# hermda02/dang

Hardware: AMD Instinct MI355X
Metric: gibbs_iterations_per_sec (higher is better)
Workload: dtype f64

## Files before the change

dang_amd/csrc/dangx_core.hip:

```cpp
#include <dlfcn.h>

#include "dx_host.h"

DxRoctx::DxRoctx() {
    const char* e = getenv("DANGX_ROCTX");
    if (!(e && e[0] == '1')) return;
    for (const char* lib : {"librocprofiler-sdk-roctx.so", "libroctx64.so"}) {
        void* h = dlopen(lib, RTLD_NOW | RTLD_GLOBAL);
        if (!h) continue;
        push = reinterpret_cast<int (*)(const char*)>(dlsym(h, "roctxRangePushA"));
        pop = reinterpret_cast<int (*)()>(dlsym(h, "roctxRangePop"));
        if (push && pop) return;
        push = nullptr; pop = nullptr;
    }
}
const DxRoctx& dx_roctx() {
    static const DxRoctx r;
    return r;
}
const char* dx_kernel_family(int kid) {
    static const char* const names[DANGX_K_COUNT] = {"dangx:amplitude_solve", "dangx:index_sweep", "dangx:sky_chisq", "dangx:reduce",
                                                     "dangx:cg_Ax", "dangx:cg_vec", "dangx:solve+sweeps", "dangx:moments", "dangx:hist",
                                                     "dangx:signal", "dangx:chains", "dangx:batches"};
    return (kid >= 0 && kid < DANGX_K_COUNT) ? names[kid] : "dangx:?";
// ... 409 lines not shown
            for (size_t q = 0; q < nbp; ++q)
                if (ctx->bp_nu0[q] != 0.0) lnr[l * nbp + q] = std::log(ctx->bp_nu0[q] / ctx->desc[l].nu_ref);
        HIPCHK(ctx, hipMemcpy(ctx->d_bp_lnr, lnr.data(), nbytes * M.ncomp, hipMemcpyHostToDevice));
        ctx->bp_dirty = false;
    }
    M.bp_nu0 = ctx->d_bp_nu0; M.bp_tau0 = ctx->d_bp_tau0;
    for (int l = 0; l < M.ncomp; ++l) {
        Comp& c = M.comp[l];
        const dangx_comp_desc& d = ctx->desc[l];
        c.type = d.type; c.nind = d.nindices; c.group = d.cg_group; c.sample_amp = d.sample_amplitude;
        c.is_synch = d.is_synch; c.nu_ref = d.nu_ref;
        c.amp = ctx->amp[l]; c.idx = ctx->idx[l];
        c.tmpl = ctx->tmpl[l]; c.corr_mask = ctx->corr_mask[l]; c.nfit = ctx->nfit[l];
        c.bp_lnr = ctx->d_bp_lnr ? ctx->d_bp_lnr + (size_t)l * nbp : nullptr;
        for (int k = 0; k < 3; ++k)
            for (int j = 0; j < MAXB; ++j) c.tamp[k][j] = ctx->tamp[l][k][j];
        if (is_global_type(c.type) && !c.tmpl) return fail(ctx, "global-amplitude component without a template map (dangx_set_template)");
        for (int q = 0; q < MAXI; ++q) {
            c.lnl_type[q] = d.lnl_type[q]; c.prior_type[q] = d.prior_type[q];
            c.gauss[q][0] = d.gauss_prior[q][0]; c.gauss[q][1] = d.gauss_prior[q][1];
            c.uni[q][0] = d.uni_prior[q][0]; c.uni[q][1] = d.uni_prior[q][1];
            c.step[q] = d.step_size[q];
            c.lgden[q] = std::log(d.gauss_prior[q][1] * std::sqrt(2.0 * PI));
        }
        c.lnuref9 = std::log(1.0 * c.nu_ref / 1.0e9);
        for (int j = 0; j < M.nbands; ++j) {
            const double nu = M.band[j].nu_c;
            const double r = nu / c.nu_ref;
            c.lnr[j] = std::log(r);
            c.lnu9[j] = std::log(1.0 * nu / 1.0e9);
            c.cst[j] = 0.0;
            if (c.type == DANGX_CMB) c.cst[j] = 1.0 / host_a2t(ctx, j);
            else if (c.type == DANGX_FREEFREE) c.cst[j] = 1.0 / (r * r);
            else if (c.type == DANGX_LOGNORMAL) { const double q = c.nu_ref / nu; c.cst[j] = q * q; }
        }
        c.const_planes = 0;
        if (c.type >= DANGX_POWERLAW && c.type <= DANGX_CMB) {
            const unsigned cp = (c.nind == 0) ? 7u : ctx->idx_const[l];
            for (int k = 0; k < M.nmaps; ++k)
                if ((cp >> k) & 1) {
                    c.const_planes |= 1 << k;
                    const double t0 = ctx->idx_val[l][k][0], t1 = ctx->idx_val[l][k][1];
                    for (int j = 0; j < M.nbands; ++j) c.csed[k][j] = dx_host_band_sed(ctx, l, j, t0, t1);
                }
        }
    }
// ... 726 lines not shown
```

dang_amd/csrc/dangx_planeset.hip:

```cpp
#ifndef DX_NO_VCOEF
#define DX_VCOEF 1
#endif
#include "dx_host.h"
#include "dx_kern_planeset.h"

static int planeset_jeff(const SweepList& sl) {
    for (int q = 0; q < sl.n; ++q) if (sl.s[q].jeff) return 1;
    return 0;
}
static size_t planeset_lds(int ng, int nb, int nv, int lanes, int Sp, int jeff, int keep = 0) {
    const int rows = (nv > Sp + jeff ? nv : Sp + jeff) + (keep ? 1 : 0);
    return ((size_t)(TROWS * ng + 3) * nb + (size_t)rows * (nb / lanes) * BLOCK) * sizeof(double);
}

static int planeset_keep(const SweepList& sl, const FusedArgs& fa, int ng, int nb, int lanes, int Sp, int bp) {
#ifdef DX_BOUNDARY_REEVAL
    return 0;
#else
    if (lanes != 1 || bp || planeset_jeff(sl)) return 0;
    const int n = sl.n < 4 ? sl.n : 4;
    for (int q = 0; q < n; ++q) {
        if (sl.s[q].mode != CH_MBB_BETA) continue;
        const int v = fa.vslot[sl.s[q].gmember];
        if (v < 0 || planeset_lds(ng, nb, fa.nv, lanes, Sp, 0, 1) > 80u * 1024u) return 0;
        return (q > 0 && v >= Sp) ? 2 : 1;
    }
    return 0;
#endif
}

static void item_codes(const SweepList& sl, int code[4]) {
    for (int q = 0; q < 4; ++q) code[q] = (q < sl.n) ? sl.s[q].mode + 8 * sl.s[q].pair + 16 * (sl.s[q].jeff ? 1 : 0) : 0;
}
static std::string planeset_name(int Sp, int nb, int ng, int lanes, int solve, const SweepList& sl, int bp) {
    int c[4];
    item_codes(sl, c);
    std::string s = "dxk::k_plane_set<" + std::to_string(Sp) + ", " + std::to_string(nb) + ", " + std::to_string(ng) + ", " + std::to_string(lanes) +
                    ", " + std::to_string(solve);
    for (int q = 0; q < 4; ++q) s += ", " + std::to_string(c[q]);
    return s + ", " + std::to_string(bp) + ">";
}

static int planeset_bp(dangx_ctx* ctx) {
    for (int j = 0; j < ctx->hm.nbands; ++j)
        if (ctx->hm.band[j].n != 0) return 1;
    return 0;
}

static bool planeset_builtin(int nb, int ng, int lanes, int solve, const SweepList& sl) {
    if (const char* e = getenv("DANGX_PLANESET_RTC"); e && e[0] == '1' && dx_rtc_enabled()) return false;
    int c[4];
    item_codes(sl, c);
    if (solve == 2)
        return lanes == 1 && nb == 10 && ng == 4 && (sl.n == 0 || (c[0] == CH_POW && c[1] == CH_MBB_BETA + 8 && c[2] == 0 && c[3] == 0));
    if (nb == 20 && ng == 6 && lanes == 2) return solve && c[0] == CH_POW && c[1] == CH_MBB_BETA + 8 && c[2] == CH_LOGN_NUP && c[3] == 0;
    if (lanes == 1 && nb == 10 && ng == 4 && solve && sl.n == 0) return true;
// ... 59 lines not shown
    return true;
}

int dx_planeset_lanes(dangx_ctx* ctx, const GroupArgs& ga, const SweepList& sl, int solve_in) {
    const int solve = planeset_solve(ga, solve_in);
    static const bool enabled = [] { const char* e = getenv("DANGX_PLANESET"); return !(e && e[0] == '0'); }();
    static const bool small_too = [] { const char* e = getenv("DANGX_PLANESET"); return !(e && e[0] == 'p'); }();
    if (!enabled || sl.n < 0 || sl.n > 4 || (sl.n == 0 && !solve) || ga.ng < 1 || ga.ng > 6) return 0;
    static const int cap2 = [] { const char* e = getenv("DANGX_PS_CAP2"); return e ? atoi(e) : 13; }();
    const int nb = ctx->hm.nbands, Sp = sl.s2 - sl.s1 + 1, cap = (Sp == 2) ? cap2 : 16;
    for (int q = 0; q < sl.n; ++q) {
        const int m = sl.s[q].mode;
        if (m < CH_POW || m > CH_LOGN_W) return 0;
        if (sl.s[q].pair && !(m == CH_MBB_BETA || m == CH_LOGN_NUP)) return 0;
        if (sl.s[q].jeff && m != CH_POW) return 0;
    }
    FusedArgs fa;
    if (!planeset_args(ctx, ga, sl, fa)) return 0;
    if (solve && fa.cal && ga.nuc > 0) return 0;
    const int bp = planeset_bp(ctx), jf = planeset_jeff(sl);
    if (bp) {
        for (int q = 0; q < sl.n; ++q)
            if (sl.s[q].mode > CH_MBB_T || sl.s[q].jeff) return 0;
        if (!(small_too && nb <= cap && planeset_lds(ga.ng, nb, fa.nv, 1, Sp, 0) <= 80u * 1024u)) return 0;
        return dx_rtc_get(ctx, "dx_kern_planeset.h", planeset_name(Sp, nb, ga.ng, 1, solve, sl, 1)) ? 1 : 0;
    }
    int lanes = 0;
    if (small_too && nb <= cap && planeset_lds(ga.ng, nb, fa.nv, 1, Sp, jf) <= 80u * 1024u) lanes = 1;
    else if (nb > 12 && nb % 2 == 0 && nb / 2 <= cap && planeset_lds(ga.ng, nb, fa.nv, 2, Sp, jf) <= 80u * 1024u) lanes = 2;
    if (!lanes) return 0;
    if (planeset_builtin(nb, ga.ng, lanes, solve, sl)) return lanes;
    return dx_rtc_get(ctx, "dx_kern_planeset.h", planeset_name(Sp, nb, ga.ng, lanes, solve, sl, 0)) ? lanes : 0;
}

bool dx_launch_planeset(dangx_ctx* ctx, const GroupArgs& ga, const SweepList& sl_in, int lanes, int solve_in, unsigned nblk, unsigned long long* accp) {
    const int solve = planeset_solve(ga, solve_in);
    FusedArgs fa;
    if (lanes < 1 || lanes > 2 || !planeset_args(ctx, ga, sl_in, fa)) return false;
    SweepList sl = sl_in;
    const int nb = ctx->hm.nbands, ng = ga.ng, Sp = sl.s2 - sl.s1 + 1;
    const int bp = planeset_bp(ctx);
    sl.keep = planeset_keep(sl, fa, ng, nb, lanes, Sp, bp);
    const size_t ldsz = planeset_lds(ng, nb, fa.nv, lanes, Sp, planeset_jeff(sl), sl.keep);
    if (!bp && planeset_builtin(nb, ng, lanes, solve, sl)) {
        if (solve == 2) dx_launch_planeset_fluct(ctx, ga, fa, sl, Sp, nblk, ldsz, accp);
        else if (planeset_jeff(sl)) dx_launch_planeset_jeff(ctx, ga, fa, sl, Sp, solve, nblk, ldsz, accp);
        else if (nb == 20) launch_builtin<20, 6, 2, 1, CH_POW, CH_MBB_BETA + 8, CH_LOGN_NUP>(ctx, ga, fa, sl, Sp, nblk, ldsz, accp);
        else if (nb == 10 && sl.n == 0) launch_builtin<10, 4, 1, 1, 0, 0, 0>(ctx, ga, fa, sl, Sp, nblk, ldsz, accp);
        else if (nb == 10 && !solve) launch_builtin<10, 4, 1, 0, CH_POW, CH_MBB_BETA + 8, 0>(ctx, ga, fa, sl, Sp, nblk, ldsz, accp);
        else if (nb == 10) launch_builtin<10, 4, 1, 1, CH_POW, CH_MBB_BETA + 8, 0>(ctx, ga, fa, sl, Sp, nblk, ldsz, accp);
        else if (nb == 5) launch_builtin<5, 3, 1, 1, CH_POW, CH_MBB_BETA + 8, 0>(ctx, ga, fa, sl, Sp, nblk, ldsz, accp);
        else launch_builtin<3, 2, 1, 1, CH_POW, CH_MBB_BETA + 8, 0>(ctx, ga, fa, sl, Sp, nblk, ldsz, accp);
        return true;
    }
    hipFunction_t fn = dx_rtc_get(ctx, "dx_kern_planeset.h", planeset_name(Sp, nb, ng, lanes, solve, sl, bp));
    if (!fn) return false;
    const Model* dm = ctx->dm;
    GroupArgs gg = ga;
    SweepList ss = sl;
    unsigned long long* bad = ctx->counters;
    double* part = ctx->partial;
    void* args[] = {&dm, &gg, &fa, &ss, &bad, &accp, &part};
    return dx_rtc_launch(ctx, fn, nblk, ldsz, args) == 0;
}

#endif
// ... 9 lines not shown
```

dang_amd/csrc/dx_chain.h:

```cpp
#pragma once
#include "dx_args.h"


template <bool V> struct BoolTag { static constexpr bool value = V; };

#ifdef DX_CHAIN_LIBEXP
#define CEXP(x) exp(x)
#define CEXPS(x) exp(x)
#define CEXPA(x) exp(x)
#define CEXP1(x) exp(x)
#else
#define CEXP(x) exp_nr(x)
#define CEXPS(x) exp_sat(x)
#define CEXPA(x) exp_any(x)
#define CEXP1(x) exp_nr_v(x)
#endif
#ifdef DX_CHAIN_IEEEDIV
#define CDIV(a, b) ((a) / (b))
#define CDIVE(a, b) ((a) / (b))
#define CRCPE(b) (1.0 / (b))
#else
#define CDIV(a, b) ((a) * fast_rcp(b))
#define CDIVE(a, b) ((a) * fast_rcp_ends(b))
#define CRCPE(b) fast_rcp_ends(b)
// ... 64 lines not shown

#ifdef DX_LNL_DIAG
__device__ unsigned long long g_lnl_diag[2];
__device__ __forceinline__ void lnl_diag_count(int k) {
    if (__lane_id() == __builtin_ctzll(__builtin_amdgcn_ballot_w64(true))) atomicAdd(&g_lnl_diag[k], 1ull);
}
#endif

template <int LP>
struct BandPick {
    int half;
    __device__ __forceinline__ double operator()(const double* arr, int j, int nbh) const {
        if (LP == 1) return arr[j];
        const double a = arr[j], b = arr[nbh + j];
        return half ? b : a;
    }
    __device__ __forceinline__ double nu_c(const Model& M, int j, int nbh) const {
        if (LP == 1) return M.band[j].nu_c;
        const double a = M.band[j].nu_c, b = M.band[nbh + j].nu_c;
        return half ? b : a;
    }
};

template <int MODE, int SP, int NB, int LP, bool KT = false, bool BP = false, bool JF = false, bool KEPT = false>
struct RegChain {
    static constexpr bool kBP = BP;
    static constexpr bool kJF = JF;
    static constexpr bool kKept = KEPT;
    static_assert(!KEPT || (LP == 1 && !BP && !JF && (MODE == CH_MBB_BETA || MODE == CH_MBB_T)), "kept factors: one-lane delta-band mbb chains");
    static_assert(!JF || (MODE == CH_POW && !BP), "Jeffreys chains: power law, delta bands");
    double D[SP][NB], F[NB], ISr[SP][NB];
    double bpa, bpb;
    double K1[(LP > 1 && !KT) ? NB : 1], K2[(LP > 1 && !KT) ? NB : 1];
    const double *kt1, *kt2;
    double amp[SP];
    double W[(JF && !KT) ? NB : 1], jS;
    double* wcol;
    const double* fcol;

    __device__ __forceinline__ double w(int j) const { return KT ? wcol[j * BLOCK] : W[j]; }
    template <class ISF>
    __device__ __forceinline__ void form_w(const Model& M, const Comp& c, ISF is_of) {
        bool bad = false;
#pragma unroll
        for (int kk = 0; kk < SP; ++kk) bad = bad || !(fabs(amp[kk]) > 0.0 && fabs(amp[kk]) < INFINITY);
#pragma unroll
        for (int j = 0; j < NB; ++j) {
            const double t0 = is_of(0, j) * is_of(0, j);
            double q = t0 * t0;
            if (SP == 2) { const double t1 = is_of(SP - 1, j) * is_of(SP - 1, j); q = fma(t1, t1, q); }
            const double l = k1(M, c, j);
            const double wj = bad ? __longlong_as_double(0x7ff8000000000000ll) : (l * l) * q;
            if (KT) wcol[j * BLOCK] = wj; else W[j] = wj;
        }
    }
    __device__ __forceinline__ void jeff_eval(const Model& M, const Comp& c, double th) {
        double S = 0.0;
#pragma unroll
        for (int j = 0; j < NB; ++j) { const double e = CEXP(th * k1(M, c, j)); S = fma(e * e, w(j), S); }
        if (LP > 1) S += __shfl_xor(S, 1, 64);
        jS = S;
    }

    __device__ __forceinline__ double is(int kk, int j) const { return ISr[kk][j]; }
    __device__ __forceinline__ void set_is(int kk, int j, double v) { ISr[kk][j] = v; }
    __device__ __forceinline__ double k1(const Model& M, const Comp& c, int j) const {
        if (KT) return kt1[j];
        if (LP > 1) return K1[j];
        return (MODE == CH_MBB_T) ? M.band[j].nu_c : (MODE == CH_LOGN_NUP) ? c.lnu9[j] : c.lnr[j];
    }
    __device__ __forceinline__ double k2(const Comp& c, int j) const { return KT ? kt2[j] : (LP > 1) ? K2[j] : c.cst[j]; }
    __device__ __forceinline__ void set_kt(const double* tab, int nbands, int ng, int g, int jb) {
        kt1 = tab + ((MODE == CH_MBB_T) ? TROWS * ng : (MODE == CH_LOGN_NUP) ? TROWS * g + 2 : TROWS * g) * nbands + jb;
        kt2 = tab + (TROWS * g + 1) * nbands + jb;
    }
    __device__ __forceinline__ void set_k(const Model& M, const Comp& c, const BandPick<LP>& pick) {
        if (LP > 1 && !KT) {
#pragma unroll
            for (int j = 0; j < NB; ++j) {
                K1[j] = (MODE == CH_MBB_T) ? pick.nu_c(M, j, NB) : (MODE == CH_LOGN_NUP) ? pick(c.lnu9, j, NB) : pick(c.lnr, j, NB);
                K2[j] = (MODE == CH_LOGN_NUP || MODE == CH_LOGN_W) ? pick(c.cst, j, NB) : 0.0;
            }
        }
    }

    template <bool BATCH, int OP = 0, bool EOUT = false>
    __device__ __forceinline__ double lnl(const Model& M, const Comp& c, double th, double other, double& acc0, double& acc1,
                                          double* eout = nullptr) {
        static_assert(!EOUT || (MODE == CH_MBB_BETA && !BP), "the exported factor is the beta chain's");
        double s0 = 0.0, s1 = 0.0;
        if (MODE == CH_POW) s0 = th;
        else if (MODE == CH_MBB_BETA) s0 = th + 1.0;
        else if (MODE == CH_MBB_T) { s0 = mbb_z(th); s1 = CEXP(s0 * c.nu_ref) - 1.0; }
        else if (MODE == CH_LOGN_NUP) { s0 = log_pos(th); s1 = other; }
        else s1 = th;
        acc0 = 0.0; acc1 = 0.0;
        double S = 0.0;
#ifdef DX_CHAIN_IEEEDIV
// ... 135 lines not shown
        else if (MODE == CH_MBB_BETA) s0 = th + 1.0;
        else { s0 = mbb_z(th); s1 = CEXP(s0 * c.nu_ref) - 1.0; }
        const double s0l = s0 * 0x1.71547652b82fep+0;
        double acc0 = 0.0, acc1 = 0.0;
#pragma unroll
        for (int j = 0; j < NB; ++j) {
            const float e = __builtin_amdgcn_exp2f((float)(s0l * k1(M, c, j)));
            double s;
            if (MODE == CH_POW) s = (double)e;
            else if (MODE == CH_MBB_BETA) s = F[j] * (double)e;
            else s = (s1 * F[j]) * (double)__builtin_amdgcn_rcpf(e - 1.0f);
            const double r0 = fma(-is(0, j), s, D[0][j]);
            acc0 = fma(r0, r0, acc0);
            if (SP == 2) {
                const double r1 = fma(-is(SP - 1, j), s, D[SP - 1][j]);
                acc1 = fma(r1, r1, acc1);
            }
        }
        double a = acc0 + acc1;
        if (LP > 1) a += __shfl_xor(a, 1, 64);
        return a;
    }

    __device__ __forceinline__ bool cheap_bound(const Model& M, const Comp& c, double lo, double hi, double a_start,
                                                double& wA, double& wG) {
        double G = 0.0, emax = 0.0, kmax = 0.0;
        double smax, zmin = 0.0;
        if (MODE == CH_POW) smax = fmax(fabs(lo), fabs(hi));
        else if (MODE == CH_MBB_BETA) smax = fmax(fabs(lo + 1.0), fabs(hi + 1.0));
        else { smax = mbb_z(lo); zmin = mbb_z(hi); }
#pragma unroll
        for (int j = 0; j < NB; ++j) {
            const double k = fabs(k1(M, c, j));
            kmax = fmax(kmax, k);
            double e;
            if (MODE == CH_MBB_T) e = (1.0 + smax * k) * 0x1p-24 + (2.0 + (double)__builtin_amdgcn_rcpf((float)(zmin * k))) * 0x1p-22;
            else e = (smax * k) * 0x1p-24 + 0x1p-22;
            e = e * (1.0 + 0x1p-8) + 0x1p-46;
            emax = fmax(emax, e);
#pragma unroll
            for (int kk = 0; kk < SP; ++kk) { const double t = e * D[kk][j]; G = fma(t, t, G); }
        }
        if (LP > 1) { G += __shfl_xor(G, 1, 64); emax = fmax(emax, __shfl_xor(emax, 1, 64)); kmax = fmax(kmax, __shfl_xor(kmax, 1, 64)); }
        const double lam = fmax(sqrt(G * fast_rcp(fmax(a_start, 0x1p-900))), 0x1p-400);
        wA = 0.5 * ((2.0 * emax * (1.0 + emax) + lam) * (1.0 + 0x1p-40) + 0x1p-40);
        wG = 0.5 * ((G * fast_rcp(lam) + 2.0 * G) * (1.0 + 0x1p-40) + 0x1p-1000);
        const bool range = smax * kmax * 0x1.71547652b82fep+0 <= 125.0;
        return (MODE == CH_MBB_T) ? (range && lo > 0.0 && zmin > 0.0) : range;
    }
    __device__ __forceinline__ void scale() {
#ifdef DX_CHAIN_SCALED
#pragma unroll
        for (int kk = 0; kk < SP; ++kk)
#pragma unroll
            for (int j = 0; j < NB; ++j) { D[kk][j] *= ISr[kk][j]; ISr[kk][j] *= amp[kk]; }
#endif
    }
};

template <int NB, int LP>
__device__ __forceinline__ void subtract_other(const Model& M, const Comp& c2, int k, double amp2, double t0, double t1,
                                               double (&Dk)[NB], const BandPick<LP>& pick) {
    if ((c2.const_planes >> (k - 1)) & 1) {
#pragma unroll
        for (int j = 0; j < NB; ++j) Dk[j] -= amp2 * pick(c2.csed[k - 1], j, NB);
        return;
    }
    const Prep pr = sed_prep(c2, t0, t1);
    switch (c2.type) {
    case DANGX_POWERLAW:
#pragma unroll
// ... 85 lines not shown
    } else if (MODE == CH_MBB_T && RC::kKept) {
    } else if (MODE == CH_MBB_BETA) {
        const double z = mbb_z(sample1);
        const double A = CEXP(z * c.nu_ref) - 1.0;
#pragma unroll
        for (int j = 0; j < NB; ++j) R.F[j] = CDIVE(A, CEXP(z * pick.nu_c(M, j, NB)) - 1.0);
        if (RC::kBP) { R.bpa = z; R.bpb = A; }
    } else if (MODE == CH_MBB_T) {
#pragma unroll
        for (int j = 0; j < NB; ++j) R.F[j] = CEXP((sample0 + 1.0) * pick(c.lnr, j, NB));
        if (RC::kBP) R.bpa = sample0 + 1.0;
    } else if (MODE == CH_LOGN_W) {
        {
            const double lp = log_pos(sample0);
#pragma unroll
            for (int j = 0; j < NB; ++j) R.F[j] = pick(c.lnu9, j, NB) - lp;
        }
    }
    const double other = first ? sample1 : sample0;
    const unsigned long long gpix = (unsigned long long)(M.pix0 + i);
    const int q = a.nind;
    const bool gauss = c.prior_type[q] == DANGX_PRIOR_GAUSSIAN;
    const double pmean = c.gauss[q][0], pstd = c.gauss[q][1], lgden = c.lgden[q];
    const double inv2v = 1.0 / (2 * (pstd * pstd));
    auto prior = [&](double v) -> double {
        if (!gauss) return 0.0;
#ifdef DX_CHAIN_IEEEDIV
        const double arg = ((v - pmean) * (v - pmean)) / (2 * (pstd * pstd));
#else
        const double arg = ((v - pmean) * (v - pmean)) * inv2v;
#endif
        return (arg > 745.0) ? -INFINITY : -arg - lgden;
    };
    auto jprior = [&](double S) -> double {
        double p = log_pos(sqrt(S));
        if (!(S >= 0x1p-1022 && S < INFINITY)) p = log(sqrt(S));
        return p;
    };
    unsigned long long nacc = 0;
    double cur = first ? sample0 : sample1;
    double a0, a1, c0, c1;
    const double step = c.step[q], lo = c.uni[q][0], hi = c.uni[q][1];
    const bool ml_opt = (a.ml_mode == DANGX_ML_OPTIMIZE);
#if defined(DX_LNL_EXACT) || !defined(DX_CHAIN_SCALED)
    constexpr bool kCert = false;
#else
    constexpr bool kCert = !RC::kBP && !JEFF && (MODE == CH_POW || MODE == CH_MBB_BETA || MODE == CH_MBB_T);
#endif
    auto chain = [&](auto batch_tag) {
        constexpr bool B = decltype(batch_tag)::value;
        double lnl;
        if (acc_in) { a0 = acc_in[0]; a1 = acc_in[1]; lnl = a0 + a1; if (JEFF) R.jeff_eval(M, c, cur); }
        else if constexpr (ADD && RC::kKept) {
            if (scol) lnl = R.lnl_add_kept(scol, a0, a1);
            else lnl = R.template lnl<B, 1>(M, c, cur, other, a0, a1);
        }
        else lnl = R.template lnl<B, ADD ? 1 : 0>(M, c, cur, other, a0, a1);
        chi[0] = -2.0 * a0; chi[1] = -2.0 * a1;
        double lnl_old = lnl + (JEFF ? jprior(R.jS) : prior(cur));
        bool cert = false, old_exact = true, sums_exact = true;
        double wA = 0.0, wG = 0.0, wold = 0.0;
        if (kCert) {
            const bool ok = R.cheap_bound(M, c, lo, hi, -2.0 * lnl, wA, wG) && !ml_opt;
            cert = __builtin_amdgcn_ballot_w64(!ok) == 0ull;
        }
        auto mh_step = [&](double prop, uint32_t u3) {
            if (prop < lo || prop > hi) return;
            if constexpr (!kCert) {
                lnl = R.template lnl<B>(M, c, prop, other, c0, c1);
                const double lnl_new = lnl + (JEFF ? jprior(R.jS) : prior(prop));
                const double diff = lnl_new - lnl_old;
                const bool acc = ml_opt ? (diff > 0.0) : mh_accept(diff, u3);
                if (acc) { cur = prop; lnl_old = lnl_new; a0 = c0; a1 = c1; ++nacc; }
            } else {
                const double pp = prior(prop);
                bool acc = false, und = true;
                double lc = 0.0, wc = 0.0;
                if (cert) {
                    const double A = R.lnl_cheap(M, c, prop);
                    lc = -0.5 * A;
                    wc = fma(wA, A, wG);
                    const double dc = (lc + pp) - lnl_old;
                    const double W = (wc + wold) * (1.0 + 0x1p-40) + 0x1p-49 * ((fabs(lc) + fabs(pp)) + fabs(lnl_old));
                    und = !mh_certain(dc - W, dc + W, u3, acc);
#ifdef DX_LNL_DIAG
                    lnl_diag_count(0);
// ... 212 lines not shown
```

dang_amd/csrc/dx_kern_planeset.h:

```cpp
#pragma once
#include "dx_kern_fused.h"

#ifndef DX_PS_WAVES
#define DX_PS_WAVES(SP, NB, LP, SOLVE, C0) (((NB) / (LP) <= 5) ? 3 : 2)
#endif

namespace dxk {

template <int V> struct ItemCode { static constexpr int value = V; };
template <bool V> struct ItemFlag { static constexpr bool value = V; };

#ifdef DX_BOUNDARY_REEVAL
#define DX_PS_SHARE(MODE, LP, BP, JF) false
#else
#define DX_PS_SHARE(MODE, LP, BP, JF) ((MODE) == CH_MBB_BETA && (LP) == 1 && !(BP) && !(JF))
#endif
template <int MODE, int PAIR, int SP, int NBL, int LP, int NG, bool FIRST, bool LAST, bool BP, bool JF, typename RFirst>
__device__ __forceinline__ void ps_item(const Model& M, const SweepList& sl, const SweepItem& it, RFirst& R0, int i, int half,
                                        int jb, int NB, const double* __restrict__ tab, const double* __restrict__ col,
                                        double& sample0, double& sample1, double chi_first[4],
                                        double chi_last[4], unsigned int* __restrict__ accepted, int slot, const double* first_acc,
                                        double* wrow, const double* fkeep, const double* skeep) {
    const Comp& c = M.comp[it.comp];
    const BandPick<LP> pick = {half};
    const int npix = M.npix;
    IndexArgs a;
    a.comp = it.comp; a.nind = it.nind; a.s1 = sl.s1; a.s2 = sl.s2; a.nsample = sl.nsample; a.ml_mode = sl.ml_mode; a.mode = MODE;
    a.bp = 0; a.others = 0u; a.jeff = 0; a.seed = sl.seed; a.stream = it.stream;
    constexpr bool SHARE = DX_PS_SHARE(MODE, LP, BP, JF);
    RegChain<MODE, SP, NBL, LP, true, BP, JF, SHARE> R;
    R.set_kt(tab, NB, NG, it.gmember, jb);
    R.fcol = fkeep;
#pragma unroll
    for (int kk = 0; kk < SP; ++kk) {
        R.amp[kk] = c.amp[(long long)(sl.s1 + kk - 1) * npix + i];
#pragma unroll
        for (int j = 0; j < NBL; ++j) { R.D[kk][j] = R0.D[kk][j]; R.ISr[kk][j] = col[(kk * NBL + j) * BLOCK] * R.amp[kk]; }
    }
    if (JF) {
        R.wcol = wrow;
        R.form_w(M, c, [&](int kk, int j) { return col[(kk * NBL + j) * BLOCK]; });
    }
    double chia[4] = {0.0, 0.0, 0.0, 0.0}, va, acc[2];
    constexpr bool HAND = SHARE && PAIR != 0;
    double ej[HAND ? NBL : 1];
    unsigned long long na = chain_finish<MODE, SP, NBL, LP, false, !FIRST, (!PAIR && !LAST), HAND>(M, a, c, R, pick, sample0, sample1, i, half, chia, &va,
                                                                                                  FIRST ? first_acc : nullptr, acc, ej, skeep);
    if (it.nind == 0) sample0 = va; else sample1 = va;
    if (FIRST) { chi_first[0] = chia[0]; chi_first[1] = chia[1]; }
    chi_last[2] = chia[2]; chi_last[3] = chia[3];
    unsigned long long nb_ = 0ull;
    if (PAIR) {
        constexpr int MODEB = (MODE == CH_MBB_BETA || MODE == CH_LOGN_NUP) ? MODE + 1 : MODE;
        RegChain<MODEB, SP, NBL, LP, true, BP, false, HAND> RB;
        RB.set_kt(tab, NB, NG, it.gmember, jb);
        if (HAND) {
#pragma unroll
            for (int j = 0; j < NBL; ++j) RB.F[j] = ej[j];
        }
#pragma unroll
        for (int kk = 0; kk < SP; ++kk) {
            RB.amp[kk] = R.amp[kk];
#pragma unroll
            for (int j = 0; j < NBL; ++j) { RB.D[kk][j] = R.D[kk][j]; RB.ISr[kk][j] = R.ISr[kk][j]; }
        }
        IndexArgs b = a;
        b.nind = it.nind + 1; b.stream = it.stream2; b.mode = MODEB;
        double chib[4] = {0.0, 0.0, 0.0, 0.0}, vb;
        nb_ = chain_finish<MODEB, SP, NBL, LP, false, false, !LAST>(M, b, c, RB, pick, sample0, sample1, i, half, chib, &vb, acc);
        if (b.nind == 0) sample0 = vb; else sample1 = vb;
        chi_last[2] = chib[2]; chi_last[3] = chib[3];
        if (!LAST) {
#pragma unroll
            for (int kk = 0; kk < SP; ++kk)
#pragma unroll
                for (int j = 0; j < NBL; ++j) R0.D[kk][j] = RB.D[kk][j];
        }
    } else if (!LAST) {
#pragma unroll
        for (int kk = 0; kk < SP; ++kk)
#pragma unroll
            for (int j = 0; j < NBL; ++j) R0.D[kk][j] = R.D[kk][j];
    }
    if (accepted) {
        const int copy = threadIdx.x & 15;
        if (na) atomicAdd(accepted + (slot << 4) + copy, (unsigned int)na);
        if (nb_) atomicAdd(accepted + ((slot + 1) << 4) + copy, (unsigned int)nb_);
    }
}

template <int SP, int NB, int NG, int LP, int SOLVE, int C0, int C1, int C2, int C3, int BP = 0>
__global__ __launch_bounds__(BLOCK, DX_PS_WAVES(SP, NB, LP, SOLVE, C0)) void k_plane_set(const Model* __restrict__ Mp, GroupArgs ga, FusedArgs fa, SweepList sl,
                                                        unsigned long long* __restrict__ not_spd, unsigned long long* __restrict__ accepted,
                                                        double* __restrict__ chi_partial) {
    constexpr int NBL = NB / LP;
    extern __shared__ double lds[];
    const Model& M = *Mp;
    const int npix = M.npix, tid = threadIdx.x;
    double* tab = lds;
    double* col = lds + (TROWS * NG + 3) * NB + tid;
    const long long t0 = (long long)blockIdx.x * BLOCK + tid;
    const long long u = t0 / LP;
    const int half = (int)(t0 % LP), jb = half * NBL;
    const bool in_range = u < npix;
    const int i = in_range ? (int)u : 0;
    const double mk = M.mask[i];
    sed_table_build(M, tab, tid, BLOCK, ga.gc, NG);
    __shared__ unsigned int acc_blk[DX_MAX_IDXSUM * 16];
    if (tid < DX_MAX_IDXSUM * 16) acc_blk[tid] = 0u;
    __syncthreads();
    double chi[4] = {0.0, 0.0, 0.0, 0.0};
    constexpr int NS0 = C0 ? 1 + ((C0 >> 3) & 1) : 0, NS1 = C1 ? 1 + ((C1 >> 3) & 1) : 0, NS2 = C2 ? 1 + ((C2 >> 3) & 1) : 0, NS3 = C3 ? 1 + ((C3 >> 3) & 1) : 0;
    constexpr int NS = NS0 + NS1 + NS2 + NS3;
    const bool live = in_range && !is_masked(mk);
    if (in_range && !live && half == 0) {
        for (int q = 0; q < sl.n; ++q) {
            const Comp& c = M.comp[sl.s[q].comp];
            for (int e = 0; e <= sl.s[q].pair; ++e) {
                double* out = c.idx + ((long long)(sl.s[q].nind + e) * M.nmaps) * npix + i;
#pragma unroll
                for (int kk = 0; kk < SP; ++kk) out[(long long)(sl.s1 + kk - 1) * npix] = 0.0;
            }
        }
    }
    if (live) {
        const long long bstride = (long long)M.nmaps * npix;
        const unsigned long long gpix = (unsigned long long)(M.pix0 + i);
        const bool sample = (ga.ml_mode == DANGX_ML_SAMPLE);
        constexpr int KQ = ((C0 & 7) == CH_MBB_BETA) ? 0 : ((C1 & 7) == CH_MBB_BETA) ? 1 : ((C2 & 7) == CH_MBB_BETA) ? 2 : 3;
        constexpr bool KEEPC = DX_PS_SHARE(CH_MBB_BETA, LP, BP, false) &&
// ... 193 lines not shown
                const SweepItem it0 = sl.s[0];
                const double* m = col + (fa.vslot[it0.gmember] * NBL) * BLOCK;
#pragma unroll
                for (int kk = 0; kk < SP; ++kk) {
                    const double a0 = M.comp[it0.comp].amp[(long long)(sl.s1 + kk - 1) * npix + i];
                    double acc = 0.0;
#pragma unroll
                    for (int j = 0; j < NBL; ++j) {
                        const double r = R0.D[kk][j];
                        acc = fma(r, r, acc);
                        R0.D[kk][j] = fma(a0 * R0.ISr[kk][j], m[j * BLOCK], r);
                    }
                    if (LP > 1) acc += __shfl_xor(acc, 1, 64);
                    first_acc[kk] = -0.5 * acc;
                }
            }
#pragma unroll
            for (int kk = 0; kk < SP; ++kk)
#pragma unroll
                for (int j = 0; j < NBL; ++j) col[(kk * NBL + j) * BLOCK] = R0.ISr[kk][j];
            __builtin_amdgcn_sched_barrier(0);
        }
        int slot = 0;
        auto run = [&](auto code_tag, auto first_tag, auto last_tag, int q) {
            constexpr int CODE = decltype(code_tag)::value;
            constexpr bool FIRST = decltype(first_tag)::value;
            constexpr bool LAST = decltype(last_tag)::value;
            if constexpr (CODE != 0) {
                const SweepItem it = sl.s[q];
                const Comp& c = M.comp[it.comp];
                double sample0, sample1, unused[4];
                load_theta(M, c, i, sl.s1, sample0, sample1);
                ps_item<(CODE & 7), ((CODE >> 3) & 1), SP, NBL, LP, NG, FIRST, LAST, (BP != 0), ((CODE >> 4) != 0)>(M, sl, it, R0, i, half, jb, NB, tab, col, sample0, sample1,
                                                                              FIRST ? chi : unused, chi, accepted ? acc_blk : nullptr, slot, first_acc,
                                                                              col + (SP * NBL) * BLOCK, (KEEPC && q == KQ) ? fkeep : nullptr,
                                                                              (KEEPC && q == KQ) ? skeep : nullptr);
                slot += 1 + ((CODE >> 3) & 1);
            }
        };
        run(ItemCode<C0>{}, ItemFlag<true>{}, ItemFlag<C1 == 0>{}, 0);
        run(ItemCode<C1>{}, ItemFlag<false>{}, ItemFlag<C2 == 0>{}, 1);
        run(ItemCode<C2>{}, ItemFlag<false>{}, ItemFlag<C3 == 0>{}, 2);
        run(ItemCode<C3>{}, ItemFlag<false>{}, ItemFlag<true>{}, 3);
    }
    if (accepted && NS > 0) {
        __syncthreads();
        if (tid < NS) {
            unsigned int v = 0u;
            for (int q = 0; q < 16; ++q) v += acc_blk[(tid << 4) + q];
            if (v != 0u) atomicAdd(accepted + tid, (unsigned long long)v);
        }
    }
    if (chi_partial) {
        double isum[NS > 0 ? NS : 1];
#pragma unroll
        for (int q = 0; q < (NS > 0 ? NS : 1); ++q) isum[q] = 0.0;
        if (live && half == 0) {
            constexpr int code[4] = {C0, C1, C2, C3};
            constexpr int first[4] = {0, NS0, NS0 + NS1, NS0 + NS1 + NS2};
#pragma unroll
            for (int q = 0; q < 4; ++q)
                if (code[q] != 0) {
                    const double* at = M.comp[sl.s[q].comp].idx + ((long long)sl.s[q].nind * M.nmaps + (sl.s1 - 1)) * npix + i;
                    isum[first[q]] = at[0];
                    if (((code[q] >> 3) & 1) != 0) isum[first[q] + 1] = at[(long long)M.nmaps * npix];
                }
// ... 19 lines not shown
```

dang_amd/csrc/dx_model.h:

```cpp
#pragma once
#include "dx_rtc_compat.h"
#ifdef __HIPCC_RTC__
#include "dangx.h"
#else
#include "../../include/dangx.h"
#endif

namespace dx {

constexpr int MAXB = DANGX_MAX_BANDS;
constexpr int MAXC = DANGX_MAX_COMPS;
constexpr int MAXI = DANGX_MAX_IND;
constexpr int MAXG = DANGX_MAX_GROUP;
constexpr int MAXT = 4;

constexpr double PI = 3.141592653589793238462643383279502884197;
constexpr double K_B = 1.3806503e-23;
constexpr double C_LIGHT = 2.99792458e8;
constexpr double MISSVAL = -1.6375e30;
constexpr double H_PLANCK = 1.0545726691251021e-34 * 2.0 * PI;

__host__ __device__ inline double mbb_z(double T) {
    const double z = H_PLANCK / (K_B * T);
    return z > 1e-4 ? 1e-4 : (z < -1e-4 ? -1e-4 : z);
}

struct Band {
    double nu_c;
    int n;
    int off;
};

struct Comp {
    int type, nind, group, sample_amp, is_synch, pad;
    double nu_ref;
    double* amp;
    double* idx;
    int lnl_type[MAXI], prior_type[MAXI];
    double gauss[MAXI][2], uni[MAXI][2], step[MAXI];
    double lgden[MAXI];
    double lnr[MAXB];
    double cst[MAXB];
    double lnu9[MAXB];
    double lnuref9;
    int const_planes, pad1;
    double csed[3][MAXB];
    const double* tmpl;
    int corr_mask, nfit;
    double tamp[3][MAXB];
    const double* bp_lnr;
};

struct Model {
    int npix, nmaps, nbands, ncomp;
    int all_delta, pad0;
    long long pix0;
    const double* sig;
    const double* rms;
    const double* mask;
    const double* bp_nu0;
    const double* bp_tau0;
    double tcmb;
    double mbb_batch_z;
// ... 10 lines not shown
```

Measured before the change: 102.2.

## Precompute per-block certification error rows in LDS and host-side prior inverse variance

Builds a per-item certification row (per-band error bounds, max error and a range verdict) once per block in shared memory using one wavefront per row, instead of every lane recomputing the bounds from the component's prior range in each chain. The per-lane cheap bound then just reads these rows, and the held K1 coefficients are copied into registers. The Gaussian prior's inverse double variance is also precomputed on the host and stored in Comp rather than divided per call. This trades extra LDS footprint, which can push configurations over the lane or LDS thresholds, and more registers for less per-lane arithmetic.

```diff
diff --git a/dang_amd/csrc/dangx_core.hip b/dang_amd/csrc/dangx_core.hip
--- a/dang_amd/csrc/dangx_core.hip
+++ b/dang_amd/csrc/dangx_core.hip
@@ -455,6 +455,7 @@
             c.uni[q][0] = d.uni_prior[q][0]; c.uni[q][1] = d.uni_prior[q][1];
             c.step[q] = d.step_size[q];
             c.lgden[q] = std::log(d.gauss_prior[q][1] * std::sqrt(2.0 * PI));
+            c.inv2v[q] = prior_inv2v(d.gauss_prior[q][1]);
         }
         c.lnuref9 = std::log(1.0 * c.nu_ref / 1.0e9);
         for (int j = 0; j < M.nbands; ++j) {
diff --git a/dang_amd/csrc/dangx_planeset.hip b/dang_amd/csrc/dangx_planeset.hip
--- a/dang_amd/csrc/dangx_planeset.hip
+++ b/dang_amd/csrc/dangx_planeset.hip
@@ -8,9 +8,19 @@
     for (int q = 0; q < sl.n; ++q) if (sl.s[q].jeff) return 1;
     return 0;
 }
-static size_t planeset_lds(int ng, int nb, int nv, int lanes, int Sp, int jeff, int keep = 0) {
+static size_t planeset_lds(int ng, int nb, int nv, int lanes, int Sp, int jeff, int ncert, int keep = 0) {
     const int rows = (nv > Sp + jeff ? nv : Sp + jeff) + (keep ? 1 : 0);
-    return ((size_t)(TROWS * ng + 3) * nb + (size_t)rows * (nb / lanes) * BLOCK) * sizeof(double);
+    return ((size_t)(TROWS * ng + 3) * nb + (size_t)ncert * cert_row_size(nb) + (size_t)rows * (nb / lanes) * BLOCK) * sizeof(double);
+}
+
+static void item_codes(const SweepList& sl, int code[4]) {
+    for (int q = 0; q < 4; ++q) code[q] = (q < sl.n) ? sl.s[q].mode + 8 * sl.s[q].pair + 16 * (sl.s[q].jeff ? 1 : 0) : 0;
+}
+static int planeset_cert(const SweepList& sl, int bp) {
+    int c[4], n = 0;
+    item_codes(sl, c);
+    for (int q = 0; q < 4; ++q) n += dxk::ps_cert_rows(c[q], bp);
+    return n;
 }
 
 static int planeset_keep(const SweepList& sl, const FusedArgs& fa, int ng, int nb, int lanes, int Sp, int bp) {
@@ -22,16 +32,13 @@
     for (int q = 0; q < n; ++q) {
         if (sl.s[q].mode != CH_MBB_BETA) continue;
         const int v = fa.vslot[sl.s[q].gmember];
-        if (v < 0 || planeset_lds(ng, nb, fa.nv, lanes, Sp, 0, 1) > 80u * 1024u) return 0;
+        if (v < 0 || planeset_lds(ng, nb, fa.nv, lanes, Sp, 0, planeset_cert(sl, bp), 1) > 80u * 1024u) return 0;
         return (q > 0 && v >= Sp) ? 2 : 1;
     }
     return 0;
 #endif
 }
 
-static void item_codes(const SweepList& sl, int code[4]) {
-    for (int q = 0; q < 4; ++q) code[q] = (q < sl.n) ? sl.s[q].mode + 8 * sl.s[q].pair + 16 * (sl.s[q].jeff ? 1 : 0) : 0;
-}
 static std::string planeset_name(int Sp, int nb, int ng, int lanes, int solve, const SweepList& sl, int bp) {
     int c[4];
     item_codes(sl, c);
@@ -137,12 +144,13 @@
     if (bp) {
         for (int q = 0; q < sl.n; ++q)
             if (sl.s[q].mode > CH_MBB_T || sl.s[q].jeff) return 0;
-        if (!(small_too && nb <= cap && planeset_lds(ga.ng, nb, fa.nv, 1, Sp, 0) <= 80u * 1024u)) return 0;
+        if (!(small_too && nb <= cap && planeset_lds(ga.ng, nb, fa.nv, 1, Sp, 0, 0) <= 80u * 1024u)) return 0;
         return dx_rtc_get(ctx, "dx_kern_planeset.h", planeset_name(Sp, nb, ga.ng, 1, solve, sl, 1)) ? 1 : 0;
     }
+    const int nc = planeset_cert(sl, 0);
     int lanes = 0;
-    if (small_too && nb <= cap && planeset_lds(ga.ng, nb, fa.nv, 1, Sp, jf) <= 80u * 1024u) lanes = 1;
-    else if (nb > 12 && nb % 2 == 0 && nb / 2 <= cap && planeset_lds(ga.ng, nb, fa.nv, 2, Sp, jf) <= 80u * 1024u) lanes = 2;
+    if (small_too && nb <= cap && planeset_lds(ga.ng, nb, fa.nv, 1, Sp, jf, nc) <= 80u * 1024u) lanes = 1;
+    else if (nb > 12 && nb % 2 == 0 && nb / 2 <= cap && planeset_lds(ga.ng, nb, fa.nv, 2, Sp, jf, nc) <= 80u * 1024u) lanes = 2;
     if (!lanes) return 0;
     if (planeset_builtin(nb, ga.ng, lanes, solve, sl)) return lanes;
     return dx_rtc_get(ctx, "dx_kern_planeset.h", planeset_name(Sp, nb, ga.ng, lanes, solve, sl, 0)) ? lanes : 0;
@@ -156,7 +164,7 @@
     const int nb = ctx->hm.nbands, ng = ga.ng, Sp = sl.s2 - sl.s1 + 1;
     const int bp = planeset_bp(ctx);
     sl.keep = planeset_keep(sl, fa, ng, nb, lanes, Sp, bp);
-    const size_t ldsz = planeset_lds(ng, nb, fa.nv, lanes, Sp, planeset_jeff(sl), sl.keep);
+    const size_t ldsz = planeset_lds(ng, nb, fa.nv, lanes, Sp, planeset_jeff(sl), planeset_cert(sl, bp), sl.keep);
     if (!bp && planeset_builtin(nb, ng, lanes, solve, sl)) {
         if (solve == 2) dx_launch_planeset_fluct(ctx, ga, fa, sl, Sp, nblk, ldsz, accp);
         else if (planeset_jeff(sl)) dx_launch_planeset_jeff(ctx, ga, fa, sl, Sp, solve, nblk, ldsz, accp);
diff --git a/dang_amd/csrc/dx_chain.h b/dang_amd/csrc/dx_chain.h
--- a/dang_amd/csrc/dx_chain.h
+++ b/dang_amd/csrc/dx_chain.h
@@ -110,21 +110,70 @@
     }
 };
 
+template <int MODE>
+__device__ __forceinline__ void cert_range(double lo, double hi, double& smax, double& zmin) {
+    zmin = 0.0;
+    if (MODE == CH_POW) smax = fmax(fabs(lo), fabs(hi));
+    else if (MODE == CH_MBB_BETA) smax = fmax(fabs(lo + 1.0), fabs(hi + 1.0));
+    else { smax = mbb_z(lo); zmin = mbb_z(hi); }
+}
+template <int MODE>
+__device__ __forceinline__ double cert_band(double smax, double zmin, double k) {
+    double e;
+    if (MODE == CH_MBB_T) e = (1.0 + smax * k) * 0x1p-24 + (2.0 + (double)__builtin_amdgcn_rcpf((float)(zmin * k))) * 0x1p-22;
+    else e = (smax * k) * 0x1p-24 + 0x1p-22;
+    return e * (1.0 + 0x1p-8) + 0x1p-46;
+}
+template <int MODE>
+__device__ __forceinline__ bool cert_verdict(double lo, double smax, double zmin, double kmax) {
+    const bool range = smax * kmax * 0x1.71547652b82fep+0 <= 125.0;
+    return (MODE == CH_MBB_T) ? (range && lo > 0.0 && zmin > 0.0) : range;
+}
+constexpr int CERT_EMAX = 0, CERT_OK = 1, CERT_TAIL = 2;
+__host__ __device__ constexpr int cert_row_size(int nb) { return nb + CERT_TAIL; }
+template <int MODE>
+__device__ __forceinline__ void cert_row_build(const Model& M, const Comp& c, int q, int nb, double* row, int tid, int wave) {
+    if ((tid >> 6) != wave) return;
+    const int lane = tid & 63;
+    const double lo = c.uni[q][0], hi = c.uni[q][1];
+    double smax, zmin;
+    cert_range<MODE>(lo, hi, smax, zmin);
+    const int j = lane < nb ? lane : nb - 1;
+    const double k = fabs((MODE == CH_MBB_T) ? M.band[j].nu_c : c.lnr[j]);
+    const double e = cert_band<MODE>(smax, zmin, k);
+    if (lane < nb) row[lane] = e;
+    double emax = e, kmax = k;
+    for (int o = 32; o > 0; o >>= 1) { emax = fmax(emax, __shfl_xor(emax, o, 64)); kmax = fmax(kmax, __shfl_xor(kmax, o, 64)); }
+    emax = fmax(emax, 0.0); kmax = fmax(kmax, 0.0);
+    if (lane == 0) {
+        row[nb + CERT_EMAX] = emax;
+        row[nb + CERT_OK] = cert_verdict<MODE>(lo, smax, zmin, kmax) ? 1.0 : 0.0;
+    }
+}
+
 template <int MODE, int SP, int NB, int LP, bool KT = false, bool BP = false, bool JF = false, bool KEPT = false>
 struct RegChain {
     static constexpr bool kBP = BP;
     static constexpr bool kJF = JF;
     static constexpr bool kKept = KEPT;
+#ifdef DX_CERT_PER_LANE
+    static constexpr bool kCertRow = false;
+#else
+    static constexpr bool kCertRow = KT;
+#endif
+    static constexpr bool kCertified = !BP && !JF && (MODE == CH_POW || MODE == CH_MBB_BETA || MODE == CH_MBB_T);
+    static constexpr bool kHeld = kCertRow && kCertified;
     static_assert(!KEPT || (LP == 1 && !BP && !JF && (MODE == CH_MBB_BETA || MODE == CH_MBB_T)), "kept factors: one-lane delta-band mbb chains");
     static_assert(!JF || (MODE == CH_POW && !BP), "Jeffreys chains: power law, delta bands");
     double D[SP][NB], F[NB], ISr[SP][NB];
     double bpa, bpb;
-    double K1[(LP > 1 && !KT) ? NB : 1], K2[(LP > 1 && !KT) ? NB : 1];
+    double K1[((LP > 1 && !KT) || kHeld) ? NB : 1], K2[(LP > 1 && !KT) ? NB : 1];
     const double *kt1, *kt2;
     double amp[SP];
     double W[(JF && !KT) ? NB : 1], jS;
     double* wcol;
     const double* fcol;
+    const double *cej, *ctail;
 
     __device__ __forceinline__ double w(int j) const { return KT ? wcol[j * BLOCK] : W[j]; }
     template <class ISF>
@@ -153,6 +202,7 @@
     __device__ __forceinline__ double is(int kk, int j) const { return ISr[kk][j]; }
     __device__ __forceinline__ void set_is(int kk, int j, double v) { ISr[kk][j] = v; }
     __device__ __forceinline__ double k1(const Model& M, const Comp& c, int j) const {
+        if (kHeld) return K1[j];
         if (KT) return kt1[j];
         if (LP > 1) return K1[j];
         return (MODE == CH_MBB_T) ? M.band[j].nu_c : (MODE == CH_LOGN_NUP) ? c.lnu9[j] : c.lnr[j];
@@ -161,7 +211,12 @@
     __device__ __forceinline__ void set_kt(const double* tab, int nbands, int ng, int g, int jb) {
         kt1 = tab + ((MODE == CH_MBB_T) ? TROWS * ng : (MODE == CH_LOGN_NUP) ? TROWS * g + 2 : TROWS * g) * nbands + jb;
         kt2 = tab + (TROWS * g + 1) * nbands + jb;
-    }
+        if (kHeld) {
+#pragma unroll
+            for (int j = 0; j < NB; ++j) K1[j] = kt1[j];
+        }
+    }
+    __device__ __forceinline__ void set_cert(const double* row, int nbands, int jb) { cej = row + jb; ctail = row + nbands; }
     __device__ __forceinline__ void set_k(const Model& M, const Comp& c, const BandPick<LP>& pick) {
         if (LP > 1 && !KT) {
 #pragma unroll
@@ -343,31 +398,40 @@
         return a;
     }
 
+    __device__ __forceinline__ void cheap_widths(double G, double emax, double a_start, double& wA, double& wG) const {
+        const double lam = fmax(sqrt(G * fast_rcp(fmax(a_start, 0x1p-900))), 0x1p-400);
+        wA = 0.5 * ((2.0 * emax * (1.0 + emax) + lam) * (1.0 + 0x1p-40) + 0x1p-40);
+        wG = 0.5 * ((G * fast_rcp(lam) + 2.0 * G) * (1.0 + 0x1p-40) + 0x1p-1000);
+    }
     __device__ __forceinline__ bool cheap_bound(const Model& M, const Comp& c, double lo, double hi, double a_start,
                                                 double& wA, double& wG) {
         double G = 0.0, emax = 0.0, kmax = 0.0;
-        double smax, zmin = 0.0;
-        if (MODE == CH_POW) smax = fmax(fabs(lo), fabs(hi));
-        else if (MODE == CH_MBB_BETA) smax = fmax(fabs(lo + 1.0), fabs(hi + 1.0));
-        else { smax = mbb_z(lo); zmin = mbb_z(hi); }
+        double smax, zmin;
+        cert_range<MODE>(lo, hi, smax, zmin);
 #pragma unroll
         for (int j = 0; j < NB; ++j) {
             const double k = fabs(k1(M, c, j));
             kmax = fmax(kmax, k);
-            double e;
-            if (MODE == CH_MBB_T) e = (1.0 + smax * k) * 0x1p-24 + (2.0 + (double)__builtin_amdgcn_rcpf((float)(zmin * k))) * 0x1p-22;
-            else e = (smax * k) * 0x1p-24 + 0x1p-22;
-            e = e * (1.0 + 0x1p-8) + 0x1p-46;
+            const double e = cert_band<MODE>(smax, zmin, k);
             emax = fmax(emax, e);
 #pragma unroll
             for (int kk = 0; kk < SP; ++kk) { const double t = e * D[kk][j]; G = fma(t, t, G); }
         }
         if (LP > 1) { G += __shfl_xor(G, 1, 64); emax = fmax(emax, __shfl_xor(emax, 1, 64)); kmax = fmax(kmax, __shfl_xor(kmax, 1, 64)); }
-        const double lam = fmax(sqrt(G * fast_rcp(fmax(a_start, 0x1p-900))), 0x1p-400);
-        wA = 0.5 * ((2.0 * emax * (1.0 + emax) + lam) * (1.0 + 0x1p-40) + 0x1p-40);
-        wG = 0.5 * ((G * fast_rcp(lam) + 2.0 * G) * (1.0 + 0x1p-40) + 0x1p-1000);
-        const bool range = smax * kmax * 0x1.71547652b82fep+0 <= 125.0;
-        return (MODE == CH_MBB_T) ? (range && lo > 0.0 && zmin > 0.0) : range;
+        cheap_widths(G, emax, a_start, wA, wG);
+        return cert_verdict<MODE>(lo, smax, zmin, kmax);
+    }
+    __device__ __forceinline__ bool cheap_bound(const double* ej, const double* tail, double a_start, double& wA, double& wG) {
+        double G = 0.0;
+#pragma unroll
+        for (int j = 0; j < NB; ++j) {
+            const double e = ej[j];
+#pragma unroll
+            for (int kk = 0; kk < SP; ++kk) { const double t = e * D[kk][j]; G = fma(t, t, G); }
+        }
+        if (LP > 1) G += __shfl_xor(G, 1, 64);
+        cheap_widths(G, tail[CERT_EMAX], a_start, wA, wG);
+        return tail[CERT_OK] != 0.0;
     }
     __device__ __forceinline__ void scale() {
 #ifdef DX_CHAIN_SCALED
@@ -499,7 +563,11 @@
     const int q = a.nind;
     const bool gauss = c.prior_type[q] == DANGX_PRIOR_GAUSSIAN;
     const double pmean = c.gauss[q][0], pstd = c.gauss[q][1], lgden = c.lgden[q];
-    const double inv2v = 1.0 / (2 * (pstd * pstd));
+#ifdef DX_CERT_PER_LANE
+    const double inv2v = prior_inv2v(pstd);
+#else
+    const double inv2v = c.inv2v[q];
+#endif
     auto prior = [&](double v) -> double {
         if (!gauss) return 0.0;
 #ifdef DX_CHAIN_IEEEDIV
@@ -522,7 +590,7 @@
 #if defined(DX_LNL_EXACT) || !defined(DX_CHAIN_SCALED)
     constexpr bool kCert = false;
 #else
-    constexpr bool kCert = !RC::kBP && !JEFF && (MODE == CH_POW || MODE == CH_MBB_BETA || MODE == CH_MBB_T);
+    constexpr bool kCert = RC::kCertified;
 #endif
     auto chain = [&](auto batch_tag) {
         constexpr bool B = decltype(batch_tag)::value;
@@ -538,7 +606,10 @@
         bool cert = false, old_exact = true, sums_exact = true;
         double wA = 0.0, wG = 0.0, wold = 0.0;
         if (kCert) {
-            const bool ok = R.cheap_bound(M, c, lo, hi, -2.0 * lnl, wA, wG) && !ml_opt;
+            bool ok;
+            if constexpr (RC::kCertRow) ok = R.cheap_bound(R.cej, R.ctail, -2.0 * lnl, wA, wG);
+            else ok = R.cheap_bound(M, c, lo, hi, -2.0 * lnl, wA, wG);
+            ok = ok && !ml_opt;
             cert = __builtin_amdgcn_ballot_w64(!ok) == 0ull;
         }
         auto mh_step = [&](double prop, uint32_t u3) {
diff --git a/dang_amd/csrc/dx_kern_planeset.h b/dang_amd/csrc/dx_kern_planeset.h
--- a/dang_amd/csrc/dx_kern_planeset.h
+++ b/dang_amd/csrc/dx_kern_planeset.h
@@ -9,6 +9,12 @@
 
 template <int V> struct ItemCode { static constexpr int value = V; };
 template <bool V> struct ItemFlag { static constexpr bool value = V; };
+
+__host__ __device__ constexpr int ps_cert_rows(int code, int bp) {
+    const int m = code & 7;
+    if (code == 0 || bp != 0 || (code >> 4) != 0 || !(m == CH_POW || m == CH_MBB_BETA || m == CH_MBB_T)) return 0;
+    return (m == CH_MBB_BETA && ((code >> 3) & 1) != 0) ? 2 : 1;
+}
 
 #ifdef DX_BOUNDARY_REEVAL
 #define DX_PS_SHARE(MODE, LP, BP, JF) false
@@ -20,7 +26,7 @@
                                         int jb, int NB, const double* __restrict__ tab, const double* __restrict__ col,
                                         double& sample0, double& sample1, double chi_first[4],
                                         double chi_last[4], unsigned int* __restrict__ accepted, int slot, const double* first_acc,
-                                        double* wrow, const double* fkeep, const double* skeep) {
+                                        double* wrow, const double* fkeep, const double* skeep, const double* crow) {
     const Comp& c = M.comp[it.comp];
     const BandPick<LP> pick = {half};
     const int npix = M.npix;
@@ -30,6 +36,7 @@
     constexpr bool SHARE = DX_PS_SHARE(MODE, LP, BP, JF);
     RegChain<MODE, SP, NBL, LP, true, BP, JF, SHARE> R;
     R.set_kt(tab, NB, NG, it.gmember, jb);
+    R.set_cert(crow, NB, jb);
     R.fcol = fkeep;
 #pragma unroll
     for (int kk = 0; kk < SP; ++kk) {
@@ -54,6 +61,7 @@
         constexpr int MODEB = (MODE == CH_MBB_BETA || MODE == CH_LOGN_NUP) ? MODE + 1 : MODE;
         RegChain<MODEB, SP, NBL, LP, true, BP, false, HAND> RB;
         RB.set_kt(tab, NB, NG, it.gmember, jb);
+        RB.set_cert(crow + cert_row_size(NB), NB, jb);
         if (HAND) {
 #pragma unroll
             for (int j = 0; j < NBL; ++j) RB.F[j] = ej[j];
@@ -97,8 +105,11 @@
     extern __shared__ double lds[];
     const Model& M = *Mp;
     const int npix = M.npix, tid = threadIdx.x;
+    constexpr int CR0 = ps_cert_rows(C0, BP), CR1 = ps_cert_rows(C1, BP), CR2 = ps_cert_rows(C2, BP), CR3 = ps_cert_rows(C3, BP);
+    constexpr int NCR = CR0 + CR1 + CR2 + CR3;
     double* tab = lds;
-    double* col = lds + (TROWS * NG + 3) * NB + tid;
+    double* cert = lds + (TROWS * NG + 3) * NB;
+    double* col = cert + NCR * cert_row_size(NB) + tid;
     const long long t0 = (long long)blockIdx.x * BLOCK + tid;
     const long long u = t0 / LP;
     const int half = (int)(t0 % LP), jb = half * NBL;
@@ -106,6 +117,21 @@
     const int i = in_range ? (int)u : 0;
     const double mk = M.mask[i];
     sed_table_build(M, tab, tid, BLOCK, ga.gc, NG);
+#ifndef DX_CERT_PER_LANE
+    auto cert_rows = [&](auto code_tag, int q, int r) {
+        constexpr int CODE = decltype(code_tag)::value;
+        if constexpr (ps_cert_rows(CODE, BP) > 0) {
+            const Comp& c = M.comp[sl.s[q].comp];
+            cert_row_build<(CODE & 7)>(M, c, sl.s[q].nind, NB, cert + r * cert_row_size(NB), tid, r % (BLOCK / 64));
+            if constexpr (ps_cert_rows(CODE, BP) > 1)
+                cert_row_build<(CODE & 7) + 1>(M, c, sl.s[q].nind + 1, NB, cert + (r + 1) * cert_row_size(NB), tid, (r + 1) % (BLOCK / 64));
+        }
+    };
+    cert_rows(ItemCode<C0>{}, 0, 0);
+    cert_rows(ItemCode<C1>{}, 1, CR0);
+    cert_rows(ItemCode<C2>{}, 2, CR0 + CR1);
+    cert_rows(ItemCode<C3>{}, 3, CR0 + CR1 + CR2);
+#endif
     __shared__ unsigned int acc_blk[DX_MAX_IDXSUM * 16];
     if (tid < DX_MAX_IDXSUM * 16) acc_blk[tid] = 0u;
     __syncthreads();
@@ -345,7 +371,7 @@
             __builtin_amdgcn_sched_barrier(0);
         }
         int slot = 0;
-        auto run = [&](auto code_tag, auto first_tag, auto last_tag, int q) {
+        auto run = [&](auto code_tag, auto first_tag, auto last_tag, int q, int crow) {
             constexpr int CODE = decltype(code_tag)::value;
             constexpr bool FIRST = decltype(first_tag)::value;
             constexpr bool LAST = decltype(last_tag)::value;
@@ -357,14 +383,14 @@
                 ps_item<(CODE & 7), ((CODE >> 3) & 1), SP, NBL, LP, NG, FIRST, LAST, (BP != 0), ((CODE >> 4) != 0)>(M, sl, it, R0, i, half, jb, NB, tab, col, sample0, sample1,
                                                                               FIRST ? chi : unused, chi, accepted ? acc_blk : nullptr, slot, first_acc,
                                                                               col + (SP * NBL) * BLOCK, (KEEPC && q == KQ) ? fkeep : nullptr,
-                                                                              (KEEPC && q == KQ) ? skeep : nullptr);
+                                                                              (KEEPC && q == KQ) ? skeep : nullptr, cert + crow * cert_row_size(NB));
                 slot += 1 + ((CODE >> 3) & 1);
             }
         };
-        run(ItemCode<C0>{}, ItemFlag<true>{}, ItemFlag<C1 == 0>{}, 0);
-        run(ItemCode<C1>{}, ItemFlag<false>{}, ItemFlag<C2 == 0>{}, 1);
-        run(ItemCode<C2>{}, ItemFlag<false>{}, ItemFlag<C3 == 0>{}, 2);
-        run(ItemCode<C3>{}, ItemFlag<false>{}, ItemFlag<true>{}, 3);
+        run(ItemCode<C0>{}, ItemFlag<true>{}, ItemFlag<C1 == 0>{}, 0, 0);
+        run(ItemCode<C1>{}, ItemFlag<false>{}, ItemFlag<C2 == 0>{}, 1, CR0);
+        run(ItemCode<C2>{}, ItemFlag<false>{}, ItemFlag<C3 == 0>{}, 2, CR0 + CR1);
+        run(ItemCode<C3>{}, ItemFlag<false>{}, ItemFlag<true>{}, 3, CR0 + CR1 + CR2);
     }
     if (accepted && NS > 0) {
         __syncthreads();
diff --git a/dang_amd/csrc/dx_model.h b/dang_amd/csrc/dx_model.h
--- a/dang_amd/csrc/dx_model.h
+++ b/dang_amd/csrc/dx_model.h
@@ -25,6 +25,8 @@
     return z > 1e-4 ? 1e-4 : (z < -1e-4 ? -1e-4 : z);
 }
 
+__host__ __device__ inline double prior_inv2v(double pstd) { return 1.0 / (2 * (pstd * pstd)); }
+
 struct Band {
     double nu_c;
     int n;
@@ -39,6 +41,7 @@
     int lnl_type[MAXI], prior_type[MAXI];
     double gauss[MAXI][2], uni[MAXI][2], step[MAXI];
     double lgden[MAXI];
+    double inv2v[MAXI];
     double lnr[MAXB];
     double cst[MAXB];
     double lnu9[MAXB];
```

After: 102.5, median of 6. No clear change (+0.3%).
